# viviendbk/ben-or-consensus-algorithm

Hardware: AMD Instinct MI355X
Metric: simulated node-rounds/sec at N=1024,F=341, 1–8 GPUs; % of INT/popcount roofline (higher is better)
Workload: dtype e2m1 0/1 votes -> f32 exact integer counts

## Files before the change

ben-or-consensus-algorithm_amd/benor/__init__.py:

```python
from __future__ import annotations

import ctypes
import os
import secrets
import struct
from typing import Sequence

_HERE = os.path.dirname(os.path.abspath(__file__))
LIB_PATH = os.environ.get("BENOR_LIB_PATH") or os.path.join(os.path.dirname(_HERE), "lib", "libbenor.so")

BO_OK = 0
BO_ERR_ARRAYS_DONT_MATCH = 1
BO_ERR_FAULTY_COUNT = 2
BO_ERR_INVALID_ARGUMENT = 3
BO_ERR_NO_DEVICE = 4
BO_ERR_HIP = 5
BO_ERR_OUT_OF_RANGE = 6
BO_ERR_UNSUPPORTED = 7
BO_ERR_ALREADY_STARTED = 8
BO_MODE_LOCKSTEP = 0
BO_MODE_RANDOM_DELIVERY = 1
BO_MODE_EVENT = 2
BO_MODE_RANDOM_TALLY = 3
BO_MODE_RANDOM_TALLY3 = 4
# ... 26 lines not shown
BO_KERNEL_TALLY_PARTIAL = 12
BO_KERNEL_TALLY_SUBSET = 13
BO_KERNEL_TALLY_BYZ = 14
KERNEL_NAMES = {BO_KERNEL_NONE: "none", BO_KERNEL_BLOCKED: "blocked popcount", BO_KERNEL_W: "W popcount",
                BO_KERNEL_RANDOM: "random delivery", BO_KERNEL_EVENT: "event level", BO_KERNEL_LANE: "lane",
                BO_KERNEL_MFMA: "matrix core (e2m1 MFMA)", BO_KERNEL_MFMA_SMALL: "packed matrix core (e2m1 MFMA, m <= 32)",
                BO_KERNEL_TALLY: "count-level random delivery (hypergeometric tallies)",
                BO_KERNEL_TALLY3: "count-level random delivery, three vote classes (hypergeometric tally + walk)",
                BO_KERNEL_TALLY_CRASH: "count-level random delivery with crashes during the run (a table per live count)",
                BO_KERNEL_TALLY_PARTIAL: "count-level random delivery with crashes cutting a broadcast short "
                                         "(a segment of receivers per cut)",
                BO_KERNEL_TALLY_SUBSET: "count-level random delivery with crashes whose last broadcast reaches a random "
                                        "subset (a reach pass per group, per-lane draws for the receivers it reaches)",
                BO_KERNEL_TALLY_BYZ: "count-level random delivery with Byzantine senders (an honest plane, wave-uniform "
                                     "steps from a staged row, per-lane Binomial lies and draws otherwise)"}
BO_MAX_N = 4096
BO_MAX_K = 1024

KNOBS = {
    "BENOR_NO_MFMA": "validation", "BENOR_NO_MFMA_BIG": "validation", "BENOR_BIG_FORM": "validation",
    "BENOR_COOP_BW": "validation", "BENOR_SMALL_MIN_TRIALS": "validation", "BENOR_BLOCKS_PER_CU": "tuning",
    "BENOR_EVENT_LANES_PER_CU": "tuning", "BENOR_TEST_DEFER_SEG_CAP": "test", "BENOR_TIMELINE": "diagnostic",
    "BENOR_EVENT_FORM": "validation", "BENOR_LIVE_WAVES": "tuning", "BENOR_EVENT_STATS": "diagnostic",
    "BENOR_MFMA_PAIR": "validation",
}

BASE_NODE_PORT = 3000
DEFAULT_K_MAX = 64

EXPORTED_SYMBOLS = (
    "bo_network_create", "bo_consensus_start", "bo_consensus_stop", "bo_node_stop",
    "bo_get_state", "bo_status", "bo_network_size", "bo_network_destroy", "bo_hist_len",
    "bo_plan_create", "bo_plan_launch", "bo_plan_run", "bo_plan_popc_words_per_node_round",
    "bo_plan_live_nodes", "bo_plan_destroy", "bo_run_trials", "bo_run_trial_states",
    "bo_popc_peak", "bo_last_error", "bo_abi_version", "bo_kernel_version", "bo_plan_kernel", "bo_kernel_for",
    "bo_mfma_peak", "bo_consensus_start_sched", "bo_plan_check",
    "bo_consensus_start_live", "bo_consensus_wait", "bo_live_stop_events", "bo_get_states", "bo_consensus_poll",
    "bo_tally_cdf", "bo_byz_cdf",
)


class Error(Exception):
    """The reference's `new Error(message)` (launchNodes.ts:11,13)."""


class AlreadyStartedError(RuntimeError):
    """libbenor error 8: a second start on one network (its inboxes persist, node.ts:29-30)."""
# ... 477 lines not shown
```

ben-or-consensus-algorithm_amd/csrc/benor_internal.h:

```cpp
#pragma once

#include <hip/hip_runtime.h>
#include <stdint.h>

#include "benor.h"

namespace benor {

constexpr uint32_t kStreamCoin = 0u;
constexpr uint32_t kStreamInit = 1u;
constexpr uint32_t kStreamDelivery = 2u;
constexpr uint32_t kStreamOrder = 3u;
constexpr uint32_t kStreamCrash = 4u;
constexpr uint32_t kStreamTally = 5u;
constexpr uint32_t kStreamWalk = 6u;
constexpr uint32_t kStreamSchedule = 7u;
constexpr uint32_t kStreamCut = 8u;
constexpr uint32_t kStreamReach = 9u;
constexpr uint32_t kStreamLie = 10u;
constexpr uint32_t kStreamHeard = 11u;

constexpr int kWavesPerBlock = 4;

constexpr uint32_t kMaxW = BO_MAX_N / 64;
constexpr int kMaxWSpecialised = 32;
constexpr uint32_t kMaxLaneM = 64;
constexpr uint32_t kMaxSmallMfmaM = 32;
constexpr uint32_t kMaxMfmaM = 1024;
// ... 52 lines not shown
  uint32_t defer_seg_cap;
  uint32_t *overflow;
  const uint64_t *ev_stops;
  uint32_t ev_nstops;
  uint32_t ev_rstops;
  uint32_t live;
  uint32_t *live_box;
  uint32_t ev_wg;
  unsigned long long *ev_stats;
  uint32_t ev_hs;
  const uint32_t *trial_list, *trial_list_len;
  uint32_t cont_round;
  unsigned long long *timeline;
  const CrashDir *cr_dir;
  const uint32_t *cr_list;
  uint32_t cr_n, cr_random;
  union {
    uint32_t cr_cut;
    uint32_t cr_reach;
  };
  const unsigned long long *byz_plane;
  const unsigned long long *byz_thr;
  uint32_t byz_n, byz_strategy, byz_one, byz_lds;
};

constexpr uint32_t kTimelineWords = 12;


constexpr uint32_t kLiveReq = 2;
constexpr uint32_t kLiveEv = kLiveReq + 128;
constexpr uint32_t kSnapReq = kLiveEv + BO_MAX_N;
constexpr uint32_t kSnapSeq = kSnapReq + 1u;
constexpr uint32_t kSnapE = kSnapSeq + 1u;
constexpr uint32_t kSnapSt = kSnapE + 4u;
constexpr uint32_t kLiveBoxWords = kSnapSt + 2u * BO_MAX_N;

constexpr uint32_t kMfmaContRounds = 3;
static_assert(16u * kMfmaContRounds <= 64u, "deferral length words overflow their block");

constexpr uint64_t kDeferChunk = 1ull << 22;

const char *knob(const char *name);
uint32_t knob_u32(const char *name, uint32_t dflt);
bool knob_is(const char *name, const char *value);

void plan_geometry(KParams &p);
// ... 46 lines not shown
hipError_t launch_event_wg(const KParams &p, int grid_blocks, hipStream_t stream);

template <int W>
hipError_t launch_w(const KParams &p, int grid_blocks, hipStream_t stream);
template <int G>
hipError_t launch_b(const KParams &p, int grid_blocks, hipStream_t stream);
template <int MM>
hipError_t launch_lane_m(const KParams &p, int grid_blocks, hipStream_t stream);

template <int MM>
hipError_t launch_mfma_small_m(const KParams &p, int grid_blocks, hipStream_t stream);
constexpr uint32_t small_slots(uint32_t m) { return (32u / m) < 8u ? (32u / m) : 8u; }
constexpr uint32_t kSmallMaxRound = 3;
constexpr uint32_t small_init_passes(uint32_t m) { return (16u * small_slots(m) + 1u + 63u) / 64u; }
constexpr uint32_t small_wave_words(uint32_t m) {
  return 7u * 64u * small_slots(m) + 64u + 256u * small_init_passes(m);
}
constexpr uint64_t kSmallMinTrials = 500000;
bool small_on_lane(const KParams &p);

template <int W>
hipError_t launch_mfma(const KParams &p, int grid_blocks, hipStream_t stream);
hipError_t launch_mfma_big(const KParams &p, int grid_blocks, hipStream_t stream);
uint32_t mfma_big_lds_bytes(const KParams &p, uint32_t block_waves);
uint32_t mfma_big_block_waves(const KParams &p);
bool mfma_big_coop(const KParams &p);
hipError_t launch_mfma_coop(const KParams &p, int grid_blocks, hipStream_t stream);
uint32_t mfma_coop_lds_bytes(const KParams &p);
uint32_t mfma_coop_block_waves(const KParams &p);
int mfma_coop_blocks_per_cu(const KParams &p);

int lockstep_grid(const KParams &p, int device);
uint32_t block_waves(const KParams &p);
uint64_t defer_units(const KParams &p, int grid);

hipError_t launch_mfma_peak(float *sink, int grid_blocks, int iters, hipStream_t stream, double *terms_per_launch);

hipError_t launch_popc_peak(uint32_t *sink, int grid_blocks, int iters, hipStream_t stream,
                            double *words_per_launch);

}
```

ben-or-consensus-algorithm_amd/csrc/benor_kernels.hip:

```cpp
#include <stdlib.h>

#include "benor_device.h"

#include <cstring>

namespace benor {

typedef __attribute__((address_space(3))) uint32_t lds_u32;

__device__ __forceinline__ lds_u32 *bitset_word(uint32_t bit, uint32_t lbase) {
  uint32_t a;
  asm("v_lshl_add_u32 %0, %1, 8, %2" : "=v"(a) : "v"(bit >> 5), "v"(lbase));
  return (lds_u32 *)(uintptr_t)a;
}

__device__ __forceinline__ void floyd_insert(uint32_t lbase, uint32_t t, uint32_t jj) {
  const uint32_t cur = *bitset_word(t, lbase);
  const uint32_t set = __builtin_amdgcn_ubfe(cur, t, 1u);
  const uint32_t idx = t + __umul24(set, jj - t);
  __hip_atomic_fetch_or(bitset_word(idx, lbase), 1u << (idx & 31u), __ATOMIC_RELAXED, __HIP_MEMORY_SCOPE_WAVEFRONT);
}

__device__ __forceinline__ void random_tally(const uint4 *__restrict__ plane, uint32_t *__restrict__ B,
                                             uint32_t W, uint32_t m, uint32_t q, bool active, uint32_t k0,
// ... 700 lines not shown
    q.variant = p.base_variant;
    q.G = p.base_G;
    return launch_lockstep(q, grid, s);
  }
  if (p.variant == 1)
    return dispatch_w(p, grid, s, std::make_integer_sequence<int, kMaxWSpecialised - 1>{});
  return dispatch_b(p, grid, s, std::make_integer_sequence<int, 12>{});
}

uint32_t block_waves(const KParams &p) {
  if (mfma_big_coop(p)) return mfma_coop_block_waves(p);
  return (p.variant == 7 && p.W > 16u && !p.node_out && !p.rounds_out) ? mfma_big_block_waves(p) : (uint32_t)kWavesPerBlock;
}

uint64_t defer_units(const KParams &p, int grid) {
  return mfma_big_coop(p) ? (uint64_t)grid : (uint64_t)grid * block_waves(p);
}

bool small_on_lane(const KParams &p) {
  if (p.node_out || p.rounds_out) return true;
  return p.trial_count < knob_u32("BENOR_SMALL_MIN_TRIALS", (uint32_t)kSmallMinTrials);
}

int lockstep_grid(const KParams &p, int device) {
  int cus = 256;
  (void)hipDeviceGetAttribute(&cus, hipDeviceAttributeMultiprocessorCount, device);
  if (p.variant == 5) {
    const uint64_t g = p.trial_count < p.ev_lanes ? p.trial_count : p.ev_lanes;
    return (int)(g < 1u ? 1u : g);
  }
  if (p.variant == 4) {
    const uint64_t blocks_needed = (p.trial_count + 255u) / 256u;
    uint64_t grid = p.ev_lanes / 256u;
    if (blocks_needed < grid) grid = blocks_needed;
    return (int)(grid < 1 ? 1 : grid);
  }
  if (p.variant == 8) {
    if (small_on_lane(p)) {
      KParams q = p;
      q.variant = p.base_variant;
      q.G = p.base_G;
      q.lds_bytes = q.hist_bytes + kWavesPerBlock * q.wave_bytes;
      return lockstep_grid(q, device);
    }
    const uint64_t batch = 64u * small_slots(p.m);
    const uint64_t groups = (p.trial_count + batch - 1u) / batch;
// ... 38 lines not shown
  }
  if (p.variant == 11) {
    const uint64_t fit = (uint64_t)crash_blocks_per_cu(p);
    if (fit >= 1u && fit < per_cu) per_cu = fit;
  }
  if (p.variant == 12) {
    const uint64_t fit = (uint64_t)partial_blocks_per_cu(p);
    if (fit >= 1u && fit < per_cu) per_cu = fit;
  }
  if (p.variant == 13) {
    const uint64_t fit = (uint64_t)subset_blocks_per_cu(p);
    if (fit >= 1u && fit < per_cu) per_cu = fit;
  }
  if (p.variant == 14) {
    const uint64_t fit = (uint64_t)byz_blocks_per_cu(p);
    if (fit >= 1u && fit < per_cu) per_cu = fit;
  }
  if (p.variant == 6) {
    const uint64_t rounds = p.G == 1u ? (p.m <= p.F ? p.k_max : 2u) : 1u;
    const uint64_t want = p.trial_count * rounds / ((uint64_t)cus * 64u * kWavesPerBlock * 8u);
    const uint64_t v = want < 2u ? 2u : want;
    if (v < per_cu) per_cu = v;
  }
  {
    const uint64_t v = knob_u32("BENOR_BLOCKS_PER_CU", 0u);
    if (v >= 1u && v < per_cu) per_cu = v;
  }
  uint64_t grid = (uint64_t)cus * per_cu;
  if (blocks_needed < grid) grid = blocks_needed;
  if (grid < 1) grid = 1;
  return (int)grid;
}

hipError_t launch_popc_peak(uint32_t *sink, int grid, int iters, hipStream_t s, double *words) {
  hipLaunchKernelGGL(popc_peak_kernel, dim3(grid), dim3(256), 0, s, sink, iters);
  if (words) *words = (double)grid * 256.0 * (double)iters * 64.0;
  return hipGetLastError();
}

}
```

ben-or-consensus-algorithm_amd/csrc/benor_mfma.h:

```cpp
#pragma once

#include "benor_device.h"
#include "benor_mfma_pair.h"

namespace benor {

typedef int mf_v4i __attribute__((ext_vector_type(4)));
typedef int mf_v8i __attribute__((ext_vector_type(8)));
typedef float mf_v16f __attribute__((ext_vector_type(16)));

template <int SA = 0>
__device__ __forceinline__ mf_v16f mfma_count(mf_v4i a, mf_v4i b, mf_v16f c) {
  const mf_v8i a8 = __builtin_shufflevector(a, a, 0, 1, 2, 3, -1, -1, -1, -1);
  const mf_v8i b8 = __builtin_shufflevector(b, b, 0, 1, 2, 3, -1, -1, -1, -1);
  return __builtin_amdgcn_mfma_scale_f32_32x32x64_f8f6f4(a8, b8, c, 4, 4, 0, 127 + SA, 0, 127);
}

__device__ __forceinline__ uint32_t sign_bytes(float e0, float e1, float e2, float e3) {
  const uint32_t lo = __builtin_amdgcn_perm(__float_as_uint(e1), __float_as_uint(e0), 0x0C0C0B09u);
  const uint32_t hi = __builtin_amdgcn_perm(__float_as_uint(e3), __float_as_uint(e2), 0x0B090C0Cu);
  return lo | hi;
}

__device__ __forceinline__ uint32_t pack_signs8(const mf_v16f &acc, int base) {
  const uint32_t s0 = sign_bytes(acc[base + 0], acc[base + 1], acc[base + 2], acc[base + 3]);
  const uint32_t s1 = sign_bytes(acc[base + 4], acc[base + 5], acc[base + 6], acc[base + 7]);
  return (s0 & 0x02020202u) | (s1 & 0x20202020u);
}

__device__ __forceinline__ uint32_t pack_fp4_8(const mf_v16f &acc, int base) {
  uint32_t r;
  asm volatile("" : "=v"(r));
// ... 15 lines not shown
  asm volatile("" : "+v"(hm));
  const uint32_t keep_a = half_sel(hm, r.y, r.x), keep_b = half_sel(hm, r.w, r.z);
  const uint32_t give_a = half_sel(hm, r.x, r.y), give_b = half_sel(hm, r.z, r.w);
  const int xa = (int)(((threadIdx.x & 63u) ^ 32u) << 2);
  const uint32_t recv_a = (uint32_t)__builtin_amdgcn_ds_bpermute(xa, (int)give_a);
  const uint32_t recv_b = (uint32_t)__builtin_amdgcn_ds_bpermute(xa, (int)give_b);
  xw[0] = half_sel(hm, recv_a, keep_a);
  xw[1] = half_sel(hm, recv_b, keep_b);
  xw[2] = half_sel(hm, keep_a, recv_a);
  xw[3] = half_sel(hm, keep_b, recv_b);
}

__device__ __forceinline__ mf_v4i expand_votes(uint32_t w) {
  return mf_v4i{(int)((w << 1) & 0x22222222u), (int)(w & 0x22222222u), (int)((w >> 1) & 0x22222222u),
                (int)((w >> 2) & 0x22222222u)};
}

__device__ __forceinline__ uint32_t pack_pair4(const mf_v16f &acc, int base) {
  const uint32_t x = __builtin_amdgcn_perm(__float_as_uint(acc[base + 1]), __float_as_uint(acc[base + 0]), pairf::kSelX);
  const uint32_t y = __builtin_amdgcn_perm(__float_as_uint(acc[base + 3]), __float_as_uint(acc[base + 2]), pairf::kSelY);
  return (x & pairf::kMaskX) | (y & pairf::kMaskY);
}

template <int W, bool HALF, int KIND, bool PAIR = false>
__global__ void __launch_bounds__(256) benor_mfma_kernel(KParams p) {
  static_assert(!PAIR || KIND == 0, "the paired form is KIND 0's");
  constexpr int MT = 2 * W - (HALF ? 1 : 0);
  constexpr int KP = (MT + 1) / 2;
  constexpr int NB = (W + 1) / 2;
  constexpr int NJ = (NB + 1) / 2;
  constexpr bool SURE = KIND == 0;
  constexpr bool PAIRED = PAIR;
  extern __shared__ __attribute__((aligned(16))) unsigned char smem[];
  const uint32_t lane = threadIdx.x & 63u, h = lane >> 5;
  const uint32_t wv = (uint32_t)__builtin_amdgcn_readfirstlane((int)(threadIdx.x >> 6));
  const uint32_t cont = SURE ? 0u : p.cont_round;
  uint32_t m = p.m, hist_len = p.hist_len;
  uint32_t trial_count = cont ? *p.trial_list_len : (uint32_t)p.trial_count;
  asm volatile("" : "+s"(m), "+s"(hist_len), "+s"(trial_count));

  uint32_t *lhist = reinterpret_cast<uint32_t *>(smem);
  uint32_t *keys = reinterpret_cast<uint32_t *>(smem + p.hist_bytes - kParamBytes);
  for (uint32_t i = threadIdx.x; i < hist_len; i += blockDim.x) lhist[i] = 0u;
  if (threadIdx.x == 0) {
    keys[0] = (uint32_t)p.seed;
    keys[1] = (uint32_t)(p.seed >> 32);
    keys[2] = (uint32_t)p.trial_begin;
    keys[3] = (uint32_t)(p.trial_begin >> 32);
  }
// ... 27 lines not shown
      const bool live = row < mrem;
      const bool live_lo = (MT & 1) ? live : true, live_hi = (MT & 1) ? false : live;
      tailq[j >> 2] |= (live_lo ? pairf::nib_lo(j & 3) : 0u) | (live_hi ? pairf::nib_hi(j & 3) : 0u);
    }
  }
  uint32_t fixed_w[W];
  if (!random_init) {
#pragma unroll
    for (int c = 0; c < W; ++c) {
      const uint4 q = p.init_plane[c];
      fixed_w[c] = h ? q.w : q.z;
    }
  }
  const int last_bits = (int)m - 32 * (2 * (W - 1) + (int)h);
  const uint32_t last_mask = last_bits >= 32 ? ~0u : (last_bits <= 0 ? 0u : ((1u << last_bits) - 1u));

  mf_v4i ones = {0x22222222, 0x22222222, 0x22222222, 0x22222222};
  uint32_t f_all = 0, f_1 = 0, f_2 = 0;
  const uint32_t ngroups = (trial_count + 31u) >> 5;
  const uint32_t waves_total = gridDim.x * kWavesPerBlock;
  const uint32_t wave_id = blockIdx.x * kWavesPerBlock + wv;
  uint32_t n_def = 0;
  uint32_t *seg = SURE ? nullptr : p.defer_seg + (size_t)wave_id * p.defer_seg_cap;
  for (uint32_t g = wave_id; g < ngroups; g += waves_total) {
    const uint32_t t = (g << 5) + (lane & 31u);
    const bool valid = t < trial_count;
    const uint32_t toff = cont ? (valid ? p.trial_list[t] : 0u) : t;
    uint32_t xw[W];
    if (SURE ? false : cont != 0u) {
      const uint64_t trial = lds_u64(keys + 2) + toff;
      const uint2 kk = lds_keys(keys);
#pragma unroll
      for (int c = 0; c < W; ++c) {
        const uint4 r = coin_block(kk.x, kk.y, (uint32_t)trial, (uint32_t)(trial >> 32), 32u * (2u * c + h), cont - 1u);
        xw[c] = coin_word(r, cont - 1u);
      }
    } else if (random_init) {
      const uint64_t trial = lds_u64(keys + 2) + t;
      const uint2 kk = lds_keys(keys);
#pragma unroll
      for (int j = 0; j < NJ; ++j) {
        const uint4 r = philox4x32_10(kk.x, kk.y,
                                      make_uint4((uint32_t)trial, (uint32_t)(trial >> 32), 2u * j + h, kStreamInit << 24));
        uint32_t q4[4];
        half_trade(r, h, q4);
#pragma unroll
        for (int q = 0; q < 4; ++q)
// ... 243 lines not shown
      }
      const bool defer = qz != 0u || (KIND == 2 && !(ma > dec_thr));
      const uint64_t bd = ballot(valid && defer);
      const uint32_t dcols = (uint32_t)bd | (uint32_t)(bd >> 32);
      halt &= ~dcols;
      if (dcols) {
        if (lane < 32u && ((dcols >> lane) & 1u)) {
          const uint32_t idx = n_def + (uint32_t)__builtin_popcount(dcols & ((1u << lane) - 1u));
          if (idx < p.defer_seg_cap) seg[idx] = toff;
        }
        n_def += (uint32_t)__builtin_popcount(dcols);
      }
      const uint64_t b1 = ballot(mx > 0.0f);
      const uint64_t b0 = ballot(mn < 0.0f);
      any1 = (uint32_t)b1 | (uint32_t)(b1 >> 32);
      any0 = (uint32_t)b0 | (uint32_t)(b0 >> 32);
    }
    any1 &= halt;
    any0 &= halt;
    f_all += (uint32_t)__builtin_popcount(halt);
    f_1 += (uint32_t)__builtin_popcount(any1);
    f_2 += (uint32_t)__builtin_popcount(any1 & any0);
  }
  if constexpr (!SURE) {
    if (n_def > p.defer_seg_cap) {
      if (lane == 0) atomicOr(p.overflow, 1u);
      n_def = p.defer_seg_cap;
    }
    uint32_t *wdef = keys + 4;
    if (lane == 0) wdef[wv] = n_def;
    __syncthreads();
    uint32_t before = 0u, total = 0u;
#pragma unroll
    for (uint32_t w = 0; w < (uint32_t)kWavesPerBlock; ++w) {
      const uint32_t c = wdef[w];
      total += c;
      before += w < wv ? c : 0u;
    }
    __syncthreads();
    if (threadIdx.x == 0 && total) wdef[0] = atomicAdd(p.defer_len, total);
    __syncthreads();
    if (n_def) {
      const uint32_t base = wdef[0] + before;
      for (uint32_t i = lane; i < n_def; i += 64u) p.defer_list[base + i] = seg[i];
    }
  }

  const uint32_t rb = 3u * (cont ? cont : 1u);
  const uint32_t hc = lane == rb ? f_all - f_1 : (lane == rb + 1u ? f_1 - f_2 : (lane == rb + 2u ? f_2 : 0u));
  if (hc) atomicAdd(&lhist[lane], hc);
  if (lane == 0 && f_2) atomicAdd(&lhist[hist_len - 1u], f_2);
  __syncthreads();
  flush_hist(lhist, p);
}

template <int W, int KIND, bool PAIR = false>
static inline void launch_mfma_kind(const KParams &p, int grid, hipStream_t s) {
  if (p.m <= 64u * (uint32_t)(W - 1) + 32u)
    hipLaunchKernelGGL((benor_mfma_kernel<W, true, KIND, PAIR>), dim3(grid), dim3(64 * kWavesPerBlock), p.hist_bytes, s, p);
  else
    hipLaunchKernelGGL((benor_mfma_kernel<W, false, KIND, PAIR>), dim3(grid), dim3(64 * kWavesPerBlock), p.hist_bytes, s, p);
}

template <int W>
static inline void launch_mfma_sure(const KParams &p, int grid, hipStream_t s) {
  if (knob_is("BENOR_MFMA_PAIR", "0")) launch_mfma_kind<W, 0, false>(p, grid, s);
  else launch_mfma_kind<W, 0, true>(p, grid, s);
}

template <int W>
hipError_t launch_mfma(const KParams &p, int grid, hipStream_t s) {
  if (p.G == 0u) launch_mfma_sure<W>(p, grid, s);
  else if (p.G == 1u) launch_mfma_kind<W, 1>(p, grid, s);
  else launch_mfma_kind<W, 2>(p, grid, s);
  return hipGetLastError();
}

}
```

ben-or-consensus-algorithm_amd/csrc/benor_mfma_02_06.hip:

```cpp
#include "benor_mfma.h"

namespace benor {
template hipError_t launch_mfma<2>(const KParams &, int, hipStream_t);
template hipError_t launch_mfma<3>(const KParams &, int, hipStream_t);
template hipError_t launch_mfma<4>(const KParams &, int, hipStream_t);
template hipError_t launch_mfma<5>(const KParams &, int, hipStream_t);
template hipError_t launch_mfma<6>(const KParams &, int, hipStream_t);
}

namespace benor {

__global__ void __launch_bounds__(256) mfma_peak_kernel(float *sink, int iters) {
  const uint32_t lane = threadIdx.x & 63u;
  mf_v4i a = {0x22222222, 0x22222222, 0x22222222, 0x22222222};
  const mf_v4i b = expand_votes(0x9E3779B9u * (lane + 1u));
  mf_v16f acc0 = {}, acc1 = {};
  for (int i = 0; i < iters; ++i) {
    asm volatile("" : "+v"(a));
    acc0 = mfma_count(a, b, acc0);
    acc1 = mfma_count(a, b, acc1);
  }
  float s = 0.f;
#pragma unroll
  for (int j = 0; j < 16; ++j) s += acc0[j] + acc1[j];
  if (s == 1.0f) sink[blockIdx.x] = s;
}

hipError_t launch_mfma_peak(float *sink, int grid, int iters, hipStream_t s, double *terms) {
  hipLaunchKernelGGL(mfma_peak_kernel, dim3(grid), dim3(256), 0, s, sink, iters);
  if (terms) *terms = (double)grid * 4.0 * 2.0 * (double)iters * 65536.0;
// ... 5 lines not shown
```

ben-or-consensus-algorithm_amd/csrc/benor_mfma_07_10.hip:

```cpp
#include "benor_mfma.h"

namespace benor {
template hipError_t launch_mfma<7>(const KParams &, int, hipStream_t);
template hipError_t launch_mfma<8>(const KParams &, int, hipStream_t);
template hipError_t launch_mfma<9>(const KParams &, int, hipStream_t);
template hipError_t launch_mfma<10>(const KParams &, int, hipStream_t);
}
```

ben-or-consensus-algorithm_amd/csrc/benor_mfma_11_13.hip:

```cpp
#include "benor_mfma.h"

namespace benor {
template hipError_t launch_mfma<11>(const KParams &, int, hipStream_t);
template hipError_t launch_mfma<12>(const KParams &, int, hipStream_t);
template hipError_t launch_mfma<13>(const KParams &, int, hipStream_t);
}
```

ben-or-consensus-algorithm_amd/csrc/benor_mfma_14_16.hip:

```cpp
#include "benor_mfma.h"

namespace benor {
template hipError_t launch_mfma<14>(const KParams &, int, hipStream_t);
template hipError_t launch_mfma<15>(const KParams &, int, hipStream_t);
template hipError_t launch_mfma<16>(const KParams &, int, hipStream_t);
}
```

ben-or-consensus-algorithm_amd/csrc/benor_runtime.cpp:

```cpp
#include <hip/hip_runtime.h>

#include <cstdio>
#include <cstring>
#include <string>
#include <algorithm>
#include <utility>
#include <cstdlib>
#include <memory>
#include <mutex>
#include <thread>
#include <chrono>
#include <cmath>
#include <vector>

#include "benor.h"
#include "benor_internal.h"

namespace {

thread_local std::string g_err;

int fail(int code, const std::string &msg) {
  g_err = msg;
  return code;
// ... 18 lines not shown
  HIP_TRY(hipGetDevice(&dev));
  hipDeviceProp_t prop;
  HIP_TRY(hipGetDeviceProperties(&prop, dev));
  if (std::strncmp(prop.gcnArchName, "gfx950", 6) != 0)
    return fail(BO_ERR_NO_DEVICE, std::string("device is ") + prop.gcnArchName + ", libbenor targets gfx950");
  if (dev_out) *dev_out = dev;
  return BO_OK;
}

__global__ void add_bin_kernel(unsigned long long *hist, uint32_t bin, unsigned long long n) {
  if (threadIdx.x == 0 && blockIdx.x == 0) hist[bin] += n;
}

}

namespace benor {
struct KnobSpec {
  const char *name, *kind;
};
constexpr KnobSpec kKnobs[] = {
    {"BENOR_NO_MFMA", "validation"},
    {"BENOR_NO_MFMA_BIG", "validation"},
    {"BENOR_MFMA_PAIR", "validation"},
    {"BENOR_BIG_FORM", "validation"},
    {"BENOR_COOP_BW", "validation"},
    {"BENOR_SMALL_MIN_TRIALS", "validation"},
    {"BENOR_BLOCKS_PER_CU", "tuning"},
    {"BENOR_EVENT_LANES_PER_CU", "tuning"},
    {"BENOR_EVENT_FORM", "validation"},
    {"BENOR_LIVE_WAVES", "tuning"},
    {"BENOR_EVENT_STATS", "diagnostic"},
    {"BENOR_TEST_DEFER_SEG_CAP", "test"},
    {"BENOR_TIMELINE", "diagnostic"},
};

const char *knob(const char *name) {
  for (const KnobSpec &k : kKnobs)
    if (std::strcmp(k.name, name) == 0) return std::getenv(name);
  std::fprintf(stderr, "libbenor: knob %s is not registered in kKnobs\n", name);
  std::abort();
}

uint32_t knob_u32(const char *name, uint32_t dflt) {
  const char *v = knob(name);
  return v && *v ? (uint32_t)std::strtoul(v, nullptr, 10) : dflt;
}
// ... 11 lines not shown
  std::vector<uint8_t> faulty;
  bool started = false;
  bool in_flight = false;
  std::shared_ptr<bo_live> live;
  int live_rc = 0;
  std::vector<uint32_t> stop_events;
  mutable std::mutex mu;
  std::mutex wait_mu;
  std::mutex snap_mu;
};

struct bo_plan {
  benor::KParams kp{};
  bo_trials_cfg cfg{};
  std::vector<uint32_t> live_ids;
  uint32_t *d_live = nullptr;
  uint4 *d_init = nullptr;
  int8_t *d_init_x = nullptr;
  uint32_t *d_crash = nullptr;
  uint32_t *d_scratch = nullptr;
  uint32_t *d_defer = nullptr;
  uint64_t defer_words = 0;
  uint32_t *d_flag = nullptr;
  uint64_t *d_stops = nullptr;
  unsigned char *d_tally = nullptr;
  int device = 0;
};

namespace {
struct LiveSlot {
  int device = -1;
  hipStream_t s = nullptr;
  uint32_t *box = nullptr;
  uint32_t *dbox = nullptr;
  unsigned char *d = nullptr;
  size_t bytes = 0;
  unsigned char *hp = nullptr;
  size_t hp_bytes = 0;
};
constexpr size_t kSlotKeepBytes = 64u << 20;
std::mutex g_slots_mu;
std::vector<LiveSlot *> g_free_slots;

struct WgRun {
  size_t o_st = 0, o_r = 0;
  size_t o_stats = 0;
// ... 484 lines not shown
  std::vector<uint4> plane;
  benor::KParams kp0;
  CrashPlan crash;
  int rc = plan_host(cfg, live, plane, kp0, live_run, &crash);
  if (rc) return rc;
  int dev = 0;
  rc = check_device(&dev);
  if (rc) return rc;

  auto *pl = new bo_plan();
  pl->cfg = *cfg;
  pl->cfg.faulty = nullptr;
  pl->cfg.init = nullptr;
  pl->cfg.crash_at = nullptr;
  pl->device = dev;
  pl->live_ids = live;
  pl->kp = kp0;
  benor::KParams &kp = pl->kp;
  const uint32_t m = kp.m;
  {
    hipError_t e = hipMalloc(&pl->d_flag, sizeof(uint32_t));
    if (e == hipSuccess) e = hipMemset(pl->d_flag, 0, sizeof(uint32_t));
    if (e != hipSuccess) { bo_plan_destroy(pl); return hip_fail(e, "plan flag"); }
  }
  if (m > 0) {
    hipError_t e = hipMalloc(&pl->d_live, sizeof(uint32_t) * m);
    if (e == hipSuccess) e = hipMalloc(&pl->d_init, sizeof(uint4) * kp.W);
    if (e == hipSuccess) e = hipMemcpy(pl->d_live, pl->live_ids.data(), sizeof(uint32_t) * m, hipMemcpyHostToDevice);
    if (e == hipSuccess) e = hipMemcpy(pl->d_init, plane.data(), sizeof(uint4) * kp.W, hipMemcpyHostToDevice);
    if (e != hipSuccess) { bo_plan_destroy(pl); return hip_fail(e, "plan upload"); }
    kp.live_ids = pl->d_live;
    kp.init_plane = pl->d_init;
    if (cfg->mode == BO_MODE_EVENT && kp.variant == 5) {
      std::vector<int8_t> ix(cfg->N, 0);
      if (cfg->init_mode == BO_INIT_FIXED)
        for (uint32_t i = 0; i < cfg->N; ++i) ix[i] = cfg->init[i];
      std::vector<uint64_t> stops;
      if (cfg->crash_at)
        for (uint32_t i = 0; i < cfg->N; ++i)
          if (cfg->crash_at[i] != 0xFFFFFFFFu) stops.push_back(((uint64_t)cfg->crash_at[i] << 12) | i);
      std::sort(stops.begin(), stops.end());
      int cus = 256;
      (void)hipDeviceGetAttribute(&cus, hipDeviceAttributeMultiprocessorCount, dev);
      const uint64_t slot = (uint64_t)kp.ev_stride * 4u;
      uint64_t slots = std::max<uint64_t>(1u, std::min<uint64_t>((uint64_t)cus, (4ull << 30) / slot));
      if (live_run) slots = 1u;
// ... 104 lines not shown
                      hipMemcpyHostToDevice);
      if (e != hipSuccess) { bo_plan_destroy(pl); return hip_fail(e, "crash tally table upload"); }
      kp.cr_dir = reinterpret_cast<const benor::CrashDir *>(pl->d_tally);
      kp.tally_off = reinterpret_cast<const uint32_t *>(pl->d_tally + dir_bytes);
      kp.cr_list = crash.list.empty() ? nullptr : reinterpret_cast<const uint32_t *>(pl->d_tally + dir_bytes + off_bytes);
      kp.tally_thr = reinterpret_cast<const unsigned long long *>(pl->d_tally + dir_bytes + off_bytes + list_bytes);
    }
  }
  *out = pl;
  return BO_OK;
}

int bo_plan_create(const bo_trials_cfg *cfg, bo_plan **out) { return plan_create_impl(cfg, out, false); }

void bo_plan_destroy(bo_plan *pl) {
  if (!pl) return;
  if (pl->d_live) (void)hipFree(pl->d_live);
  if (pl->d_init) (void)hipFree(pl->d_init);
  if (pl->d_init_x) (void)hipFree(pl->d_init_x);
  if (pl->d_crash) (void)hipFree(pl->d_crash);
  if (pl->d_scratch) (void)hipFree(pl->d_scratch);
  if (pl->d_defer) (void)hipFree(pl->d_defer);
  if (pl->d_flag) (void)hipFree(pl->d_flag);
  if (pl->d_stops) (void)hipFree(pl->d_stops);
  if (pl->d_tally) (void)hipFree(pl->d_tally);
  delete pl;
}

uint32_t bo_plan_live_nodes(const bo_plan *pl) { return pl ? pl->kp.m : 0u; }

int bo_plan_kernel(const bo_plan *pl) {
  if (!pl) return -BO_ERR_INVALID_ARGUMENT;
  return kernel_family(pl->kp);
}

uint64_t bo_plan_popc_words_per_node_round(const bo_plan *pl) {
  if (!pl) return 0;
  uint64_t counts = 4ull;
  if (pl->kp.mode != BO_MODE_RANDOM_DELIVERY && pl->kp.mode != BO_MODE_RANDOM_TALLY &&
      pl->kp.mode != BO_MODE_RANDOM_TALLY3 && pl->kp.mode != BO_MODE_CRASH_TALLY &&
      pl->kp.mode != BO_MODE_CRASH_PARTIAL && pl->kp.mode != BO_MODE_CRASH_SUBSET &&
      pl->kp.mode != BO_MODE_BYZ_TALLY)
    counts = ((pl->kp.m - pl->kp.init_q) & 1u) ? 2ull : 3ull;
  return counts * ((pl->kp.m + 31ull) / 32ull);
}

static hipError_t launch_with_timeline(benor::KParams kp, int grid, hipStream_t s, const char *path) {
  const size_t words = (size_t)grid * benor::kWavesPerBlock * benor::kTimelineWords;
  unsigned long long *d = nullptr;
  hipError_t e = hipMalloc(&d, words * sizeof(unsigned long long));
  if (e != hipSuccess) return e;
  e = hipMemsetAsync(d, 0, words * sizeof(unsigned long long), s);
  kp.timeline = d;
  if (e == hipSuccess) e = benor::launch_lockstep(kp, grid, s);
  std::vector<unsigned long long> h(words);
  if (e == hipSuccess) e = hipStreamSynchronize(s);
  if (e == hipSuccess) e = hipMemcpy(h.data(), d, words * sizeof(unsigned long long), hipMemcpyDeviceToHost);
  (void)hipFree(d);
  if (e != hipSuccess) return e;
  if (FILE *f = std::fopen(path, "a")) {
    std::fprintf(f, "# launch m=%u trials=%llu grid=%d waves=%d\n", kp.m, (unsigned long long)kp.trial_count, grid,
                 grid * benor::kWavesPerBlock);
    for (size_t w = 0; w < (size_t)grid * benor::kWavesPerBlock; ++w) {
      const unsigned long long *t = h.data() + w * benor::kTimelineWords;
      std::fprintf(f, "%zu", w);
      for (uint32_t i = 0; i < 11u; ++i) std::fprintf(f, ",%llu", t[i]);
      std::fprintf(f, "\n");
    }
    std::fclose(f);
  }
  return hipSuccess;
}

static int plan_launch_impl(bo_plan *pl, uint64_t trial_begin, uint64_t trial_count, uint64_t *hist_dev,
                            bo_node_state *node_out, uint32_t *rounds_out, hipStream_t s) {
  if (trial_count == 0) return BO_OK;
  benor::KParams kp = pl->kp;
  if (kp.m == 0) {
    hipLaunchKernelGGL(add_bin_kernel, dim3(1), dim3(64), 0, s,
                       reinterpret_cast<unsigned long long *>(hist_dev), 2u, (unsigned long long)trial_count);
    HIP_TRY(hipGetLastError());
    return BO_OK;
  }
  kp.hist = reinterpret_cast<unsigned long long *>(hist_dev);
  kp.overflow = pl->d_flag;
// ... 48 lines not shown
        }
        kc.defer_list = lists[(r - 1u) & 1u];
        kc.defer_len = lens + 16u * (r - 1u);
        kc.defer_seg_cap = (uint32_t)seg_cap_of(benor::defer_units(kc, g));
        if (test_seg_cap) kc.defer_seg_cap = std::min<uint32_t>(kc.defer_seg_cap, test_seg_cap);
        HIP_TRY(benor::launch_lockstep(kc, g, s));
        r_last = r;
      }
      benor::KParams kw = kp;
      kw.variant = kp.base_variant;
      kw.G = kp.base_G;
      kw.defer_list = kw.defer_len = kw.defer_seg = nullptr;
      kw.trial_list = lists[(r_last - 1u) & 1u];
      kw.trial_list_len = lens + 16u * (r_last - 1u);
      HIP_TRY(benor::launch_lockstep(kw, benor::lockstep_grid(kw, pl->device), s));
      done += n;
    }
    return BO_OK;
  }
  for (uint64_t done = 0; done < trial_count;) {
    const uint64_t n = std::min<uint64_t>(trial_count - done, benor::kMaxTrialsPerLaunch);
    kp.trial_begin = trial_begin + done;
    kp.trial_count = n;
    const int grid = benor::lockstep_grid(kp, pl->device);
    const char *tl_path = kp.variant == 8 ? benor::knob("BENOR_TIMELINE") : nullptr;
    if (tl_path) {
      HIP_TRY(launch_with_timeline(kp, grid, s, tl_path));
    } else {
      HIP_TRY(benor::launch_lockstep(kp, grid, s));
    }
    done += n;
  }
  return BO_OK;
}

int bo_plan_launch(bo_plan *pl, uint64_t trial_begin, uint64_t trial_count, uint64_t *hist_dev, void *stream) {
  if (!pl || !hist_dev) return fail(BO_ERR_INVALID_ARGUMENT, "NULL argument");
  return plan_launch_impl(pl, trial_begin, trial_count, hist_dev, nullptr, nullptr,
                          reinterpret_cast<hipStream_t>(stream));
}

namespace {
int plan_flag_read(bo_plan *pl, hipStream_t s, uint32_t &v);
int plan_flag_error(uint32_t v);
}

int bo_plan_run(bo_plan *pl, uint64_t trial_begin, uint64_t trial_count, uint64_t *hist_host) {
  if (!pl || !hist_host) return fail(BO_ERR_INVALID_ARGUMENT, "NULL argument");
// ... 17 lines not shown
}

namespace {
int plan_flag_read(bo_plan *pl, hipStream_t s, uint32_t &v) {
  v = 0;
  if (!pl->d_flag) return BO_OK;
  int cur = 0;
  HIP_TRY(hipGetDevice(&cur));
  if (cur != pl->device) HIP_TRY(hipSetDevice(pl->device));
  hipError_t e = hipMemcpyAsync(&v, pl->d_flag, sizeof v, hipMemcpyDeviceToHost, s);
  if (e == hipSuccess) e = hipStreamSynchronize(s);
  if (e == hipSuccess && v) e = hipMemsetAsync(pl->d_flag, 0, sizeof v, s);
  if (e == hipSuccess && v) e = hipStreamSynchronize(s);
  if (cur != pl->device) (void)hipSetDevice(cur);
  if (e != hipSuccess) return hip_fail(e, "plan flag read");
  return BO_OK;
}

int plan_flag_error(uint32_t v) {
  if (!v) return BO_OK;
  if (v & 1u)
    return fail(BO_ERR_INTERNAL, "a matrix-core launch deferred more trials than its segment holds: "
                                 "its histogram is incomplete (deferral segment sizing)");
  return fail(BO_ERR_INTERNAL, "an event-level message pool filled up: the affected trials stopped early");
}
}

int bo_plan_check(bo_plan *pl) {
  if (!pl) return fail(BO_ERR_INVALID_ARGUMENT, "NULL argument");
  if (!pl->d_flag) return BO_OK;
  int cur = 0;
  HIP_TRY(hipGetDevice(&cur));
  if (cur != pl->device) HIP_TRY(hipSetDevice(pl->device));
  const hipError_t e = hipDeviceSynchronize();
  if (cur != pl->device) (void)hipSetDevice(cur);
  if (e != hipSuccess) return hip_fail(e, "bo_plan_check");
  uint32_t v = 0;
  const int rc = plan_flag_read(pl, nullptr, v);
  return rc ? rc : plan_flag_error(v);
}

int bo_run_trials(const bo_trials_cfg *cfg, uint64_t trial_begin, uint64_t trial_count, uint64_t *hist_host) {
  bo_plan *pl = nullptr;
  int rc = bo_plan_create(cfg, &pl);
  if (rc) return rc;
  rc = bo_plan_run(pl, trial_begin, trial_count, hist_host);
// ... 503 lines not shown
```

Baseline: 3163 billion.

## Add dynamic chunked work claiming for paired MFMA kernel with occupancy-sized grid

Replaces the static grid-stride loop over trial groups in the paired MFMA kernel with dynamic work stealing. Each wave claims chunks of groups through a global atomic counter and prefetches its next claim, so faster waves take more work and tail imbalance shrinks. The grid is sized to full occupancy from the occupancy API, and a last-arriver check resets the counter and flags skipped or repeated groups. This adds per-chunk atomic traffic and a host-side occupancy query, and it only turns on when a heuristic finds enough groups per resident wave.

```diff
diff --git a/ben-or-consensus-algorithm_amd/benor/__init__.py b/ben-or-consensus-algorithm_amd/benor/__init__.py
--- a/ben-or-consensus-algorithm_amd/benor/__init__.py
+++ b/ben-or-consensus-algorithm_amd/benor/__init__.py
@@ -72,7 +72,7 @@
     "BENOR_COOP_BW": "validation", "BENOR_SMALL_MIN_TRIALS": "validation", "BENOR_BLOCKS_PER_CU": "tuning",
     "BENOR_EVENT_LANES_PER_CU": "tuning", "BENOR_TEST_DEFER_SEG_CAP": "test", "BENOR_TIMELINE": "diagnostic",
     "BENOR_EVENT_FORM": "validation", "BENOR_LIVE_WAVES": "tuning", "BENOR_EVENT_STATS": "diagnostic",
-    "BENOR_MFMA_PAIR": "validation",
+    "BENOR_MFMA_PAIR": "validation", "BENOR_MFMA_DYNAMIC": "validation", "BENOR_MFMA_CHUNK": "tuning",
 }
 
 BASE_NODE_PORT = 3000
diff --git a/ben-or-consensus-algorithm_amd/csrc/benor_internal.h b/ben-or-consensus-algorithm_amd/csrc/benor_internal.h
--- a/ben-or-consensus-algorithm_amd/csrc/benor_internal.h
+++ b/ben-or-consensus-algorithm_amd/csrc/benor_internal.h
@@ -4,6 +4,7 @@
 #include <stdint.h>
 
 #include "benor.h"
+#include "benor_mfma_sched.h"
 
 namespace benor {
 
@@ -102,6 +103,8 @@
   const unsigned long long *byz_plane;
   const unsigned long long *byz_thr;
   uint32_t byz_n, byz_strategy, byz_one, byz_lds;
+  uint32_t *mfma_claim;
+  uint32_t mfma_chunk;
 };
 
 constexpr uint32_t kTimelineWords = 12;
@@ -194,6 +197,9 @@
 template <int W>
 hipError_t launch_mfma(const KParams &p, int grid_blocks, hipStream_t stream);
 hipError_t launch_mfma_big(const KParams &p, int grid_blocks, hipStream_t stream);
+template <int W>
+int mfma_sure_blocks_per_cu(const KParams &p);
+uint32_t mfma_chunk(const KParams &p, int device);
 uint32_t mfma_big_lds_bytes(const KParams &p, uint32_t block_waves);
 uint32_t mfma_big_block_waves(const KParams &p);
 bool mfma_big_coop(const KParams &p);
diff --git a/ben-or-consensus-algorithm_amd/csrc/benor_kernels.hip b/ben-or-consensus-algorithm_amd/csrc/benor_kernels.hip
--- a/ben-or-consensus-algorithm_amd/csrc/benor_kernels.hip
+++ b/ben-or-consensus-algorithm_amd/csrc/benor_kernels.hip
@@ -746,6 +746,43 @@
   return p.trial_count < knob_u32("BENOR_SMALL_MIN_TRIALS", (uint32_t)kSmallMinTrials);
 }
 
+template <int... Is>
+static int dispatch_mfma_blocks(const KParams &p, std::integer_sequence<int, Is...>) {
+  int n = 0;
+  (void)((p.W == (uint32_t)(Is + 2) ? (n = mfma_sure_blocks_per_cu<Is + 2>(p), true) : false) || ...);
+  return n;
+}
+
+static uint32_t mfma_resident_per_cu(const KParams &p) {
+  struct Last {
+    uint32_t W, m, lds, v;
+  };
+  static thread_local Last last = {0u, 0u, 0u, 0u};
+  if (last.v && last.W == p.W && last.m == p.m && last.lds == p.hist_bytes) return last.v;
+  const int n = dispatch_mfma_blocks(p, std::make_integer_sequence<int, 15>{});
+  const uint32_t v = n >= 1 && n <= 8 ? (uint32_t)n : 8u;
+  last = Last{p.W, p.m, p.hist_bytes, v};
+  return v;
+}
+
+uint32_t mfma_chunk(const KParams &p, int device) {
+  if (p.variant != 7 || p.G != 0u || p.W > 16u || p.node_out || p.rounds_out) return 0u;
+  const bool forced = knob_is("BENOR_MFMA_DYNAMIC", "1");
+  if (knob_is("BENOR_MFMA_DYNAMIC", "0") || knob_is("BENOR_MFMA_PAIR", "0")) return 0u;
+  int cus = 256;
+  (void)hipDeviceGetAttribute(&cus, hipDeviceAttributeMultiprocessorCount, device);
+  const uint32_t MT = 2u * p.W - (p.m <= 64u * (p.W - 1u) + 32u ? 1u : 0u);
+  const uint64_t ngroups = (p.trial_count + 31u) / 32u;
+  sched::Rule r = sched::rule(p.W, MT, ngroups, 0u);
+  if (!forced && r.chunk > sched::kMaxChunk) return 0u;
+  r = sched::rule(p.W, MT, ngroups, (uint64_t)mfma_resident_per_cu(p) * (uint64_t)cus * kWavesPerBlock);
+  if (!forced && !r.dynamic) return 0u;
+  uint32_t c = r.chunk < sched::kMaxChunk ? r.chunk : sched::kMaxChunk;
+  const uint32_t v = knob_u32("BENOR_MFMA_CHUNK", 0u);
+  if (v >= 1u && v <= 64u) c = v;
+  return c;
+}
+
 int lockstep_grid(const KParams &p, int device) {
   int cus = 256;
   (void)hipDeviceGetAttribute(&cus, hipDeviceAttributeMultiprocessorCount, device);
@@ -830,9 +867,11 @@
     const uint64_t v = want < 2u ? 2u : want;
     if (v < per_cu) per_cu = v;
   }
+  const bool mfma_small_w = mfma && p.W <= 16u;
+  if (mfma_small_w && p.mfma_chunk) per_cu = mfma_resident_per_cu(p);
   {
     const uint64_t v = knob_u32("BENOR_BLOCKS_PER_CU", 0u);
-    if (v >= 1u && v < per_cu) per_cu = v;
+    if (mfma_small_w ? v >= 1u && v <= 16u : v >= 1u && v < per_cu) per_cu = v;
   }
   uint64_t grid = (uint64_t)cus * per_cu;
   if (blocks_needed < grid) grid = blocks_needed;
diff --git a/ben-or-consensus-algorithm_amd/csrc/benor_mfma.h b/ben-or-consensus-algorithm_amd/csrc/benor_mfma.h
--- a/ben-or-consensus-algorithm_amd/csrc/benor_mfma.h
+++ b/ben-or-consensus-algorithm_amd/csrc/benor_mfma.h
@@ -2,12 +2,15 @@
 
 #include "benor_device.h"
 #include "benor_mfma_pair.h"
+#include "benor_mfma_sched.h"
 
 namespace benor {
 
 typedef int mf_v4i __attribute__((ext_vector_type(4)));
 typedef int mf_v8i __attribute__((ext_vector_type(8)));
 typedef float mf_v16f __attribute__((ext_vector_type(16)));
+
+constexpr int kHwRegHwId = 4 | (31 << 11), kHwRegXccId = 20 | (31 << 11);
 
 template <int SA = 0>
 __device__ __forceinline__ mf_v16f mfma_count(mf_v4i a, mf_v4i b, mf_v16f c) {
@@ -69,9 +72,28 @@
   return (x & pairf::kMaskX) | (y & pairf::kMaskY);
 }
 
-template <int W, bool HALF, int KIND, bool PAIR = false>
+struct ClaimWords {
+  uint32_t *w;
+  __device__ __forceinline__ uint32_t claim(uint32_t C) {
+    auto q = (__attribute__((address_space(1))) uint32_t *)w;
+    asm volatile("" : "+v"(q));
+    return __hip_atomic_fetch_add(q, C, __ATOMIC_RELAXED, __HIP_MEMORY_SCOPE_AGENT);
+  }
+  __device__ __forceinline__ uint32_t arrive() {
+    return __hip_atomic_fetch_add(w + sched::kDoneWord, 1u, __ATOMIC_ACQ_REL, __HIP_MEMORY_SCOPE_AGENT);
+  }
+  __device__ __forceinline__ uint32_t take_next() {
+    return __hip_atomic_exchange(w, 0u, __ATOMIC_RELAXED, __HIP_MEMORY_SCOPE_AGENT);
+  }
+  __device__ __forceinline__ void clear_done() {
+    __hip_atomic_store(w + sched::kDoneWord, 0u, __ATOMIC_RELAXED, __HIP_MEMORY_SCOPE_AGENT);
+  }
+};
+
+template <int W, bool HALF, int KIND, bool PAIR = false, bool DYN = false>
 __global__ void __launch_bounds__(256) benor_mfma_kernel(KParams p) {
   static_assert(!PAIR || KIND == 0, "the paired form is KIND 0's");
+  static_assert(!DYN || PAIR, "dynamic claims are the paired form's");
   constexpr int MT = 2 * W - (HALF ? 1 : 0);
   constexpr int KP = (MT + 1) / 2;
   constexpr int NB = (W + 1) / 2;
@@ -145,7 +167,27 @@
   const uint32_t wave_id = blockIdx.x * kWavesPerBlock + wv;
   uint32_t n_def = 0;
   uint32_t *seg = SURE ? nullptr : p.defer_seg + (size_t)wave_id * p.defer_seg_cap;
-  for (uint32_t g = wave_id; g < ngroups; g += waves_total) {
+  unsigned long long *tl = p.timeline ? p.timeline + (size_t)wave_id * kTimelineWords : nullptr;
+  if (tl && lane == 0u) tl[0] = (unsigned long long)wall_clock64();
+  [[maybe_unused]] ClaimWords cw{p.mfma_claim};
+  [[maybe_unused]] const uint32_t C = DYN ? p.mfma_chunk : 0u;
+  [[maybe_unused]] uint32_t pending = 0u, g_end = 0u, n_run = 0u, n_claims = 0u;
+  if constexpr (DYN) {
+    if (lane == 0u) pending = sched::claim(cw, C);
+  }
+  for (uint32_t g = DYN ? 0u : wave_id; DYN || g < ngroups; g += DYN ? 1u : waves_total) {
+    if constexpr (DYN) {
+      if (g == g_end) {
+        asm volatile("" : "+v"(pending));
+        const uint32_t base = (uint32_t)__builtin_amdgcn_readfirstlane((int)pending);
+        if (base >= ngroups) break;
+        g = base;
+        g_end = sched::chunk_end(base, ngroups, C);
+        n_run += g_end - base;
+        ++n_claims;
+        if (lane == 0u) pending = sched::claim(cw, C);
+      }
+    }
     const uint32_t t = (g << 5) + (lane & 31u);
     const bool valid = t < trial_count;
     const uint32_t toff = cont ? (valid ? p.trial_list[t] : 0u) : t;
@@ -435,6 +477,20 @@
     f_1 += (uint32_t)__builtin_popcount(any1);
     f_2 += (uint32_t)__builtin_popcount(any1 & any0);
   }
+  if (tl && lane == 0u) {
+    tl[1] = (unsigned long long)wall_clock64();
+    if constexpr (!DYN) n_run = wave_id < ngroups ? (ngroups - wave_id + waves_total - 1u) / waves_total : 0u;
+    const uint32_t hw = __builtin_amdgcn_s_getreg(kHwRegHwId), xcc = __builtin_amdgcn_s_getreg(kHwRegXccId);
+    tl[2] = n_run;
+    tl[3] = xcc & 0xFu;
+    tl[4] = (hw >> 13) & 0x7u;
+    tl[5] = (hw >> 8) & 0x1Fu;
+    tl[6] = hw;
+    tl[7] = n_claims;
+  }
+  if constexpr (DYN) {
+    if (lane == 0u && !sched::finish(cw, ngroups, waves_total, C)) atomicOr(p.overflow, sched::kInvariantBit);
+  }
   if constexpr (!SURE) {
     if (n_def > p.defer_seg_cap) {
       if (lane == 0) atomicOr(p.overflow, 1u);
@@ -467,18 +523,30 @@
   flush_hist(lhist, p);
 }
 
-template <int W, int KIND, bool PAIR = false>
+template <int W, int KIND, bool PAIR = false, bool DYN = false>
 static inline void launch_mfma_kind(const KParams &p, int grid, hipStream_t s) {
   if (p.m <= 64u * (uint32_t)(W - 1) + 32u)
-    hipLaunchKernelGGL((benor_mfma_kernel<W, true, KIND, PAIR>), dim3(grid), dim3(64 * kWavesPerBlock), p.hist_bytes, s, p);
+    hipLaunchKernelGGL((benor_mfma_kernel<W, true, KIND, PAIR, DYN>), dim3(grid), dim3(64 * kWavesPerBlock), p.hist_bytes, s, p);
   else
-    hipLaunchKernelGGL((benor_mfma_kernel<W, false, KIND, PAIR>), dim3(grid), dim3(64 * kWavesPerBlock), p.hist_bytes, s, p);
+    hipLaunchKernelGGL((benor_mfma_kernel<W, false, KIND, PAIR, DYN>), dim3(grid), dim3(64 * kWavesPerBlock), p.hist_bytes, s, p);
 }
 
 template <int W>
 static inline void launch_mfma_sure(const KParams &p, int grid, hipStream_t s) {
   if (knob_is("BENOR_MFMA_PAIR", "0")) launch_mfma_kind<W, 0, false>(p, grid, s);
+  else if (p.mfma_chunk && p.mfma_claim) launch_mfma_kind<W, 0, true, true>(p, grid, s);
   else launch_mfma_kind<W, 0, true>(p, grid, s);
+}
+
+template <int W>
+int mfma_sure_blocks_per_cu(const KParams &p) {
+  int n = 0;
+  const hipError_t e =
+      p.m <= 64u * (uint32_t)(W - 1) + 32u
+          ? hipOccupancyMaxActiveBlocksPerMultiprocessor(&n, benor_mfma_kernel<W, true, 0, true, true>, 64 * kWavesPerBlock, p.hist_bytes)
+          : hipOccupancyMaxActiveBlocksPerMultiprocessor(&n, benor_mfma_kernel<W, false, 0, true, true>, 64 * kWavesPerBlock, p.hist_bytes);
+  if (e != hipSuccess) (void)hipGetLastError();
+  return e == hipSuccess ? n : 0;
 }
 
 template <int W>
diff --git a/ben-or-consensus-algorithm_amd/csrc/benor_mfma_02_06.hip b/ben-or-consensus-algorithm_amd/csrc/benor_mfma_02_06.hip
--- a/ben-or-consensus-algorithm_amd/csrc/benor_mfma_02_06.hip
+++ b/ben-or-consensus-algorithm_amd/csrc/benor_mfma_02_06.hip
@@ -2,10 +2,15 @@
 
 namespace benor {
 template hipError_t launch_mfma<2>(const KParams &, int, hipStream_t);
+template int mfma_sure_blocks_per_cu<2>(const KParams &);
 template hipError_t launch_mfma<3>(const KParams &, int, hipStream_t);
+template int mfma_sure_blocks_per_cu<3>(const KParams &);
 template hipError_t launch_mfma<4>(const KParams &, int, hipStream_t);
+template int mfma_sure_blocks_per_cu<4>(const KParams &);
 template hipError_t launch_mfma<5>(const KParams &, int, hipStream_t);
+template int mfma_sure_blocks_per_cu<5>(const KParams &);
 template hipError_t launch_mfma<6>(const KParams &, int, hipStream_t);
+template int mfma_sure_blocks_per_cu<6>(const KParams &);
 }
 
 namespace benor {
diff --git a/ben-or-consensus-algorithm_amd/csrc/benor_mfma_07_10.hip b/ben-or-consensus-algorithm_amd/csrc/benor_mfma_07_10.hip
--- a/ben-or-consensus-algorithm_amd/csrc/benor_mfma_07_10.hip
+++ b/ben-or-consensus-algorithm_amd/csrc/benor_mfma_07_10.hip
@@ -2,7 +2,11 @@
 
 namespace benor {
 template hipError_t launch_mfma<7>(const KParams &, int, hipStream_t);
+template int mfma_sure_blocks_per_cu<7>(const KParams &);
 template hipError_t launch_mfma<8>(const KParams &, int, hipStream_t);
+template int mfma_sure_blocks_per_cu<8>(const KParams &);
 template hipError_t launch_mfma<9>(const KParams &, int, hipStream_t);
+template int mfma_sure_blocks_per_cu<9>(const KParams &);
 template hipError_t launch_mfma<10>(const KParams &, int, hipStream_t);
+template int mfma_sure_blocks_per_cu<10>(const KParams &);
 }
diff --git a/ben-or-consensus-algorithm_amd/csrc/benor_mfma_11_13.hip b/ben-or-consensus-algorithm_amd/csrc/benor_mfma_11_13.hip
--- a/ben-or-consensus-algorithm_amd/csrc/benor_mfma_11_13.hip
+++ b/ben-or-consensus-algorithm_amd/csrc/benor_mfma_11_13.hip
@@ -2,6 +2,9 @@
 
 namespace benor {
 template hipError_t launch_mfma<11>(const KParams &, int, hipStream_t);
+template int mfma_sure_blocks_per_cu<11>(const KParams &);
 template hipError_t launch_mfma<12>(const KParams &, int, hipStream_t);
+template int mfma_sure_blocks_per_cu<12>(const KParams &);
 template hipError_t launch_mfma<13>(const KParams &, int, hipStream_t);
+template int mfma_sure_blocks_per_cu<13>(const KParams &);
 }
diff --git a/ben-or-consensus-algorithm_amd/csrc/benor_mfma_14_16.hip b/ben-or-consensus-algorithm_amd/csrc/benor_mfma_14_16.hip
--- a/ben-or-consensus-algorithm_amd/csrc/benor_mfma_14_16.hip
+++ b/ben-or-consensus-algorithm_amd/csrc/benor_mfma_14_16.hip
@@ -2,6 +2,9 @@
 
 namespace benor {
 template hipError_t launch_mfma<14>(const KParams &, int, hipStream_t);
+template int mfma_sure_blocks_per_cu<14>(const KParams &);
 template hipError_t launch_mfma<15>(const KParams &, int, hipStream_t);
+template int mfma_sure_blocks_per_cu<15>(const KParams &);
 template hipError_t launch_mfma<16>(const KParams &, int, hipStream_t);
+template int mfma_sure_blocks_per_cu<16>(const KParams &);
 }
diff --git a/ben-or-consensus-algorithm_amd/csrc/benor_mfma_sched.h b/ben-or-consensus-algorithm_amd/csrc/benor_mfma_sched.h
--- /dev/null
+++ b/ben-or-consensus-algorithm_amd/csrc/benor_mfma_sched.h
@@ -0,0 +1,71 @@
+#pragma once
+
+#include <stdint.h>
+
+#if defined(__HIPCC__) || defined(__CUDACC__)
+#define BENOR_SCHED_HD __host__ __device__ inline
+#else
+#define BENOR_SCHED_HD inline
+#endif
+
+namespace benor {
+namespace sched {
+
+constexpr uint32_t kMaxChunk = 16;
+constexpr uint32_t kInvariantBit = 4u;
+constexpr uint32_t kDoneWord = 32;
+constexpr uint32_t kWords = 64;
+
+struct Rule {
+  bool dynamic;
+  uint32_t chunk;
+};
+
+BENOR_SCHED_HD uint32_t groups_per_us(uint32_t W, uint32_t MT) {
+  const uint32_t KP = (MT + 1u) / 2u;
+  return 1024u * 2250u / (32u * MT * (W + KP));
+}
+
+BENOR_SCHED_HD Rule rule(uint32_t W, uint32_t MT, uint64_t ngroups, uint64_t resident_waves) {
+  const uint32_t c = (groups_per_us(W, MT) + 19u) / 20u;
+  Rule r;
+  r.chunk = c < 1u ? 1u : c;
+  r.dynamic = r.chunk <= kMaxChunk && ngroups >= 4ull * r.chunk * resident_waves;
+  return r;
+}
+
+BENOR_SCHED_HD uint32_t expected_next(uint32_t ngroups, uint32_t waves, uint32_t C) {
+  return C * ((ngroups + C - 1u) / C + waves);
+}
+
+BENOR_SCHED_HD uint32_t chunk_end(uint32_t base, uint32_t ngroups, uint32_t C) {
+  return ngroups - base < C ? ngroups : base + C;
+}
+
+template <class A>
+BENOR_SCHED_HD uint32_t claim(A &a, uint32_t C) {
+  return a.claim(C);
+}
+
+template <class A>
+BENOR_SCHED_HD bool finish(A &a, uint32_t ngroups, uint32_t waves, uint32_t C) {
+  if (a.arrive() != waves - 1u) return true;
+  const uint32_t n = a.take_next();
+  a.clear_done();
+  return n == expected_next(ngroups, waves, C);
+}
+
+template <class A, class Body>
+inline bool wave_run(A &a, uint32_t ngroups, uint32_t waves, uint32_t C, Body body) {
+  uint32_t pending = claim(a, C);
+  for (;;) {
+    const uint32_t base = pending;
+    if (base >= ngroups) break;
+    pending = claim(a, C);
+    for (uint32_t g = base, e = chunk_end(base, ngroups, C); g < e; ++g) body(g);
+  }
+  return finish(a, ngroups, waves, C);
+}
+
+}
+}
diff --git a/ben-or-consensus-algorithm_amd/csrc/benor_runtime.cpp b/ben-or-consensus-algorithm_amd/csrc/benor_runtime.cpp
--- a/ben-or-consensus-algorithm_amd/csrc/benor_runtime.cpp
+++ b/ben-or-consensus-algorithm_amd/csrc/benor_runtime.cpp
@@ -64,6 +64,8 @@
     {"BENOR_NO_MFMA", "validation"},
     {"BENOR_NO_MFMA_BIG", "validation"},
     {"BENOR_MFMA_PAIR", "validation"},
+    {"BENOR_MFMA_DYNAMIC", "validation"},
+    {"BENOR_MFMA_CHUNK", "tuning"},
     {"BENOR_BIG_FORM", "validation"},
     {"BENOR_COOP_BW", "validation"},
     {"BENOR_SMALL_MIN_TRIALS", "validation"},
@@ -121,6 +123,7 @@
   uint32_t *d_defer = nullptr;
   uint64_t defer_words = 0;
   uint32_t *d_flag = nullptr;
+  uint32_t *d_claim = nullptr;
   uint64_t *d_stops = nullptr;
   unsigned char *d_tally = nullptr;
   int device = 0;
@@ -651,6 +654,12 @@
     hipError_t e = hipMalloc(&pl->d_flag, sizeof(uint32_t));
     if (e == hipSuccess) e = hipMemset(pl->d_flag, 0, sizeof(uint32_t));
     if (e != hipSuccess) { bo_plan_destroy(pl); return hip_fail(e, "plan flag"); }
+  }
+  if (kp.variant == 7 && kp.G == 0u && kp.W <= 16u) {
+    hipError_t e = hipMalloc(&pl->d_claim, sizeof(uint32_t) * benor::sched::kWords);
+    if (e == hipSuccess) e = hipMemset(pl->d_claim, 0, sizeof(uint32_t) * benor::sched::kWords);
+    if (e != hipSuccess) { bo_plan_destroy(pl); return hip_fail(e, "plan claim words"); }
+    kp.mfma_claim = pl->d_claim;
   }
   if (m > 0) {
     hipError_t e = hipMalloc(&pl->d_live, sizeof(uint32_t) * m);
@@ -801,6 +810,7 @@
   if (pl->d_scratch) (void)hipFree(pl->d_scratch);
   if (pl->d_defer) (void)hipFree(pl->d_defer);
   if (pl->d_flag) (void)hipFree(pl->d_flag);
+  if (pl->d_claim) (void)hipFree(pl->d_claim);
   if (pl->d_stops) (void)hipFree(pl->d_stops);
   if (pl->d_tally) (void)hipFree(pl->d_tally);
   delete pl;
@@ -838,8 +848,10 @@
   (void)hipFree(d);
   if (e != hipSuccess) return e;
   if (FILE *f = std::fopen(path, "a")) {
-    std::fprintf(f, "# launch m=%u trials=%llu grid=%d waves=%d\n", kp.m, (unsigned long long)kp.trial_count, grid,
+    std::fprintf(f, "# launch m=%u trials=%llu grid=%d waves=%d", kp.m, (unsigned long long)kp.trial_count, grid,
                  grid * benor::kWavesPerBlock);
+    if (kp.variant == 7) std::fprintf(f, " kernel=mfma chunk=%u", kp.mfma_chunk);
+    std::fprintf(f, "\n");
     for (size_t w = 0; w < (size_t)grid * benor::kWavesPerBlock; ++w) {
       const unsigned long long *t = h.data() + w * benor::kTimelineWords;
       std::fprintf(f, "%zu", w);
@@ -934,8 +946,10 @@
     const uint64_t n = std::min<uint64_t>(trial_count - done, benor::kMaxTrialsPerLaunch);
     kp.trial_begin = trial_begin + done;
     kp.trial_count = n;
+    kp.mfma_chunk = benor::mfma_chunk(kp, pl->device);
     const int grid = benor::lockstep_grid(kp, pl->device);
-    const char *tl_path = kp.variant == 8 ? benor::knob("BENOR_TIMELINE") : nullptr;
+    const bool mfma_sure = kp.variant == 7 && kp.G == 0u && kp.W <= 16u && !node_out && !rounds_out;
+    const char *tl_path = kp.variant == 8 || mfma_sure ? benor::knob("BENOR_TIMELINE") : nullptr;
     if (tl_path) {
       HIP_TRY(launch_with_timeline(kp, grid, s, tl_path));
     } else {
@@ -999,6 +1013,9 @@
   if (v & 1u)
     return fail(BO_ERR_INTERNAL, "a matrix-core launch deferred more trials than its segment holds: "
                                  "its histogram is incomplete (deferral segment sizing)");
+  if (v & benor::sched::kInvariantBit)
+    return fail(BO_ERR_INTERNAL, "a matrix-core launch ended with its claim counter off: "
+                                 "groups were skipped or run twice (benor_mfma_sched.h)");
   return fail(BO_ERR_INTERNAL, "an event-level message pool filled up: the affected trials stopped early");
 }
 }
```

Result: faster. 3276 billion (median of 6 runs) (+3.6%).
